# marcusrussi/approximateNN

Hardware: AMD Instinct MI355X
Metric: queries/sec, N=10M d=128 k=10 Q=10k float (query(): hash + candidate gather + L2 + top-k + refine) (higher is better)
Workload: dtype f32; 1 GPU; cfg3: N=10000000 d=128 k=10 tries=10 Q=10000/step float; streams=1, d_short=20, L1=6006, P1=4096, L2=110, P2=64, sum_par_maxes=286

## Files before the change

### approximatenn_amd/_lib.py

```python
import ctypes as C
import os
import subprocess
import threading

CSRC = os.path.join(os.path.dirname(os.path.abspath(__file__)), "csrc")
_libs = {}


class SaveT(C.Structure):
    _fields_ = [("tries", C.c_int), ("n", C.c_size_t), ("k", C.c_size_t),
                ("d_short", C.c_size_t), ("d_long", C.c_size_t),
                ("which_par", C.POINTER(C.POINTER(C.c_size_t))),
                ("par_maxes", C.POINTER(C.c_size_t)), ("graph", C.POINTER(C.c_size_t)),
                ("row_means", C.c_void_p), ("bases", C.c_void_p)]


def build(verbose=False):
    cmd = ["make", "-j4", "-C", CSRC, "all"]
    if not verbose:
        cmd.insert(1, "-s")
    subprocess.check_call(cmd)


def reload_env():
# ... 120 lines not shown
    lib.annhip_stream_open.restype = vp
    lib.annhip_stream_open.argtypes = [vp, sz, C.c_int]
    lib.annhip_stream_submit.restype = C.c_long
    lib.annhip_stream_submit.argtypes = [vp, sz, vp, C.c_int]
    lib.annhip_stream_collect.restype = C.c_int
    lib.annhip_stream_collect.argtypes = [vp, C.c_long, vp, vp]
    lib.annhip_stream_close.argtypes = [vp]
    lib.annhip_key_bytes.restype = sz
    lib.annhip_key_bytes.argtypes = []
    lib.annhip_stream_create_reserving.restype = vp
    lib.annhip_stream_create_reserving.argtypes = [C.c_int]
    lib.annhip_stream_destroy.argtypes = [vp]
    lib.annhip_sh_codes.argtypes = [vp, vp, sz, vp, sz, sz, u32p]
    lib.annhip_sh_stage1.argtypes = [vp, vp, sz, vp, C.c_int, u32p, vp, u32p, u32p]
    lib.annhip_sh_merge_finalize.argtypes = [vp, vp, C.c_int, sz, sz, sz, vp, u32p, u32p, vp]
    lib.annhip_sh_exact1_begin.argtypes = [vp, vp, sz, vp, C.c_int, u32p, u32p, sz, u32p, u32p, vp]
    lib.annhip_sh_exact1_end.argtypes = [vp, vp, sz, sz, sz, sz, u32p, u32p, vp, u32p, vp, u32p, vp]
    lib.annhip_sh_stage2.argtypes = [vp, vp, sz, vp, C.c_int, u32p, vp, u32p]
    lib.annhip_sh_final.argtypes = [vp, vp, C.c_int, sz, sz, sz, u32p, vp, vp, u32p, vp]
    lib.annhip_stage1_rows.argtypes = [vp, sz, vp, C.c_int, u32p, u32p, sz, u32p, vp]
    lib.annhip_stage2_rows_list.argtypes = [vp, sz, vp, C.c_int, u32p, sz, u32p, vp, u32p, vp]
    lib.annhip_exact_select.argtypes = [vp, C.c_int, sz, u32p, vp, u32p, u32p, vp]
    lib.annhip_test_sort_rows.argtypes = [sz, sz, sz, u32p, vp, vp, u32p, u32p, vp, vp, C.c_int]
    lib.annhip_recall_ranks.argtypes = [sz, sz, sz, vp, sz, vp, vp, C.c_int, vp]
    lib.annhip_recall_ranks_host.argtypes = [sz, sz, sz, vp, sz, vp, vp, C.c_int, vp]
    lib.annhip_exact_knn.restype = C.c_int
    lib.annhip_exact_knn.argtypes = [sz, sz, sz, vp, sz, vp, C.c_int, vp, vp]
    lib.annhip_exact_knn_filtered.restype = C.c_int
    lib.annhip_exact_knn_filtered.argtypes = [sz, sz, sz, vp, sz, vp, C.c_int, u32p, vp, vp]
    lib.annhip_exact_knn_tagged.restype = C.c_int
    lib.annhip_exact_knn_tagged.argtypes = [sz, sz, sz, vp, sz, vp, C.c_int, vp, vp, vp, vp, vp, vp]
    lib.annhip_index_exact_query_tagged.restype = C.c_int
    lib.annhip_index_exact_query_tagged.argtypes = [vp, sz, vp, C.c_int, vp, vp, vp, vp]
    lib.annhip_exact_knn_host.restype = C.c_int
    lib.annhip_exact_knn_host.argtypes = [sz, sz, sz, vp, sz, vp, C.c_int, vp, vp]
    lib.annhip_index_exact_query.restype = C.c_int
    lib.annhip_index_exact_query.argtypes = [vp, sz, vp, C.c_int, vp, vp]
    lib.annhip_checksum_dev.restype = C.c_ulonglong
    lib.annhip_checksum_dev.argtypes = [vp, sz, vp]
    lib.annhip_index_checksum.restype = C.c_ulonglong
    lib.annhip_index_checksum.argtypes = [vp]
    lib.annhip_profile.argtypes = [vp, C.c_int]
    lib.annhip_stats.argtypes = [vp, C.POINTER(C.c_double * 8), C.c_int]
    lib.annhip_stage_ms.argtypes = [vp, C.POINTER(C.c_double * 6)]
    lib.annhip_cache_clear.argtypes = []
    lib.annhip_fingerprint_ms.restype = C.c_double
# ... 19 lines not shown
    lib.query_gpu.argtypes = [C.POINTER(SaveT), vp, sz, vp, C.POINTER(vp)]
    lib.precomp_gpu.restype = C.POINTER(sz)
    lib.precomp_gpu.argtypes = [sz, sz, sz, vp, C.c_int, sz, sz, sz, sz, C.POINTER(SaveT), C.POINTER(vp)]
    _libs[prec] = lib
    return lib


EXPORTED = ["gpu_init", "gpu_cleanup", "register_cleanup", "query_gpu", "precomp_gpu", "annhip_precision", "annhip_layout_code",
            "annhip_index_create", "annhip_index_destroy", "annhip_index_info", "annhip_index_set_stream", "annhip_index_set_gather_pieces", "annhip_index_set_gather_slots", "annhip_index_set_fixed",
            "annhip_index_set_rows", "annhip_index_rows", "annhip_index_set_prune", "annhip_index_prune",
            "annhip_index_set_probe", "annhip_index_probe", "annhip_probe_bits",
            "annhip_index_set_filter", "annhip_index_filter_count", "annhip_filter_pack", "annhip_exact_knn_filtered",
            "annhip_index_set_tags", "annhip_index_has_tags", "annhip_query_tagged", "annhip_exact_knn_tagged",
            "annhip_index_exact_query_tagged",
            "annhip_query_k", "annhip_index_max_query_k", "annhip_index_exact_query_k",
            "annhip_query_radius", "annhip_index_exact_query_radius", "annhip_radius_trim",
            "annhip_rerank", "annhip_index_rerank",
            "annhip_index_append", "annhip_index_reserve_tail", "annhip_index_tail", "annhip_index_copy_rows", "annhip_index_drop_tail",
            "annhip_index_hash_tail", "annhip_index_tail_hashed",
            "annhip_index_fixed", "annhip_index_copy_words",
            "annhip_index_export", "annhip_index_reshard", "annhip_save_write", "annhip_save_read", "annhip_precomp_index", "annhip_precomp_begin", "annhip_precomp_info", "annhip_precomp_init_merged", "annhip_precomp_hash",
            "annhip_precomp_try", "annhip_precomp_merge", "annhip_precomp_graph", "annhip_precomp_finish", "annhip_query", "annhip_workspace_create", "annhip_workspace_destroy", "annhip_query_on", "annhip_query_slice", "annhip_stream_open", "annhip_stream_submit", "annhip_stream_collect", "annhip_stream_close",
            "annhip_key_bytes", "annhip_stream_create_reserving", "annhip_stream_destroy", "annhip_sh_codes", "annhip_sh_stage1", "annhip_sh_merge_finalize", "annhip_sh_exact1_begin", "annhip_sh_exact1_end", "annhip_sh_stage2",
            "annhip_sh_final", "annhip_stage1_rows", "annhip_stage2_rows_list", "annhip_exact_select", "annhip_test_sort_rows",
            "annhip_recall_ranks", "annhip_recall_ranks_host", "annhip_exact_knn", "annhip_exact_knn_host", "annhip_index_exact_query", "annhip_checksum_dev", "annhip_index_checksum", "annhip_profile", "annhip_stats", "annhip_stage_ms",
            "annhip_cache_clear", "annhip_fingerprint_ms", "annhip_cache_drop", "annhip_cache_size", "annhip_reload_env",
            "annhip_synth_randnorm", "annhip_synth_reset", "annhip_host_profile", "annhip_host_stats",
            "annhip_host_shards", "annhip_host_stats_shard", "annhip_set_devices"]
DISPATCH_EXPORTED = ["precomp", "query", "free_save"]


_libc = C.CDLL("libc.so.6")
_libc.initstate.restype = C.c_void_p
_libc.initstate.argtypes = [C.c_uint, C.c_void_p, C.c_size_t]
_libc.setstate.restype = C.c_void_p
_libc.setstate.argtypes = [C.c_void_p]
_RAND_WORDS = (1, 8, 16, 32, 64)
_restored = []


_park_lock = threading.Lock()
_park_depth = 0
_park_old = None


class park_random:

# ... 33 lines not shown
```

### approximatenn_amd/csrc/ann_host.hip

```cpp
#include <hip/hip_fp16.h>
#include <hip/hip_runtime.h>
#include <math.h>
#include <stdio.h>
#include <stdlib.h>
#include <string.h>
#include <time.h>

#include <algorithm>
#include <limits>
#include <mutex>
#include <vector>

#include "../../include/algg.h"
#include "../../include/ann_hip.h"
#include "../../include/gpu_comp.h"
#include "ann_hostpool.h"
#include "ann_precomp_kernels.h"
#include "ann_query_kernels.h"
#include "ann_probe_kernels.h"
#include "ann_recall_kernels.h"
#include "ann_exact_kernels.h"
#include "ann_filter_kernels.h"
#include "ann_tag_kernels.h"
#include "ann_kq_kernels.h"
// ... 978 lines not shown
      if constexpr (D <= 0) {
        allow_lds(codes_kernel<D>, smem);
        hipLaunchKernelGGL(codes_kernel<D>, dim3(grid), dim3(64 * wpb), smem, s, P, (int)Q, y, codes, zero_me);
      }
    });
  }
  HIPCHECK(hipGetLastError());
}

static int stage1_waves(u32 P1, double own_frac) {
  int w = (int)(P1 / ANN_S1_CHUNK);
  if (w < 1) w = 1;
  if (w > 4) w = 4;
  if (own_frac <= 0.5) w = 1;
  if (env().s1_waves) w = env().s1_waves;
  return w;
}
static int stage1_cap(int W, int K1) {
  int cap = 256;
  if (cap < W * K1) cap = W * K1;
  if (cap < K1 + 128) cap = K1 + 128;
  return (cap + 63) & ~63;
}
static size_t stage1_lds_bytes(const QParams &P, int W, int K1, int cap, u32 tail_len = 0) {
  size_t b = sizeof(Key) * (size_t)W * cap + 2 * sizeof(Key) * (size_t)W * K1 + sizeof(TryInfo) * (size_t)P.T +
             sizeof(u32 *) * (size_t)W * ANN_WAVE + sizeof(u32) * (size_t)W * ANN_S1_CHUNK +
             sizeof(u32) * (size_t)W * ANN_WAVE + sizeof(u32) * (size_t)P.T + sizeof(int) * (size_t)W + sizeof(u32) * 4 +
             3 * sizeof(u32) * (size_t)tail_len;
  b = (b + 15) & ~(size_t)15;
  b += sizeof(FT) * (size_t)tail_len;
  b = (b + 15) & ~(size_t)15;
  if (d_needs_lds_row(P.d)) b += sizeof(FT) * (size_t)P.d * (1 + W);
  return b;
}

__global__ void zero_u32_kernel(u32 *p) { *p = 0; }

__global__ void sum_u32_kernel(size_t count, const u32 *__restrict__ v, unsigned long long *out) {
  unsigned long long acc = 0;
  for (size_t e = (size_t)blockIdx.x * blockDim.x + threadIdx.x; e < count; e += (size_t)gridDim.x * blockDim.x)
    acc += v[e];
#pragma unroll
  for (int s = 32; s >= 1; s >>= 1) acc += __shfl_xor(acc, s);
  if (lane_id() == 0) atomicAdd(out, acc);
}

static EventPair s1_prof_begin(annhip_index *ix, hipStream_t s) {
  EventPair ev;
// ... 2 lines not shown
    HIPCHECK(hipEventCreate(&ev.b));
  } else {
    ev = ix->ev_free.back();
    ix->ev_free.pop_back();
  }
  HIPCHECK(hipEventRecord(ev.a, s));
  return ev;
}
static void s1_prof_end(annhip_index *ix, EventPair ev, size_t Q, const u32 *nvo, hipStream_t s) {
  HIPCHECK(hipEventRecord(ev.b, s));
  ix->ev_used.push_back(ev);
  if (ix->profile == 1) sum_u32_kernel<<<grid_for(Q, 256, 64), 256, 0, s>>>(Q, nvo, ix->d_rows);
}

static void launch_stage1(annhip_index *ix, const QParams &P, size_t Q, const FT *y, int alias,
                          const u32 *codes, FT *cand_d, u32 *cand_i, u32 *nvt, u32 *nvo, hipStream_t s,
                          const std::vector<TryInfo> &h_tries, int use_seg, FusedTail F = FusedTail{0, 0, NULL, NULL, NULL, NULL, NULL, NULL, NULL},
                          Key *cand_key = NULL, int pieces = 1, int slots = 0, size_t qstride = 0, int keys = 0,
                          bool bracket = true) {
  const int kq = (int)(qstride ? qstride : Q);
  if (!Q) return;
  if (keys && F.enabled) die("launch_stage1: a preselection has no fused tail");
  const int K1 = keys ? keys : P.k + 1, W = stage1_waves(P.P1, (double)(P.hi - P.lo) / (double)P.n), cap = stage1_cap(W, K1);
  const size_t smem = stage1_lds_bytes(P, W, K1, cap, F.enabled == 1 ? F.len2 : 0);
  u32 runs_used = 0;
  for (int t = 0; t < P.T; t++)
    for (int yy = 0; yy <= P.ds; yy++)
      if (h_tries[t].off + (u32)yy * h_tries[t].pm < P.P1) runs_used++;
  unsigned max_grid = 0xFFFFFFFFu;
  if (slots > 0) max_grid = std::max(1u, (unsigned)device_cus() * 4u * (unsigned)slots / (unsigned)W);
  EventPair ev;
  const bool prof = ix && ix->profile && bracket;
  if (prof) ev = s1_prof_begin(ix, s);
  const size_t np = (size_t)std::max(1, std::min(pieces, 64)), per = (Q + np - 1) / np;
  with_value(QueryLayouts{}, layout_code(P.d), [&](auto dd) {
    with_rows(P, [&](auto rt) {
      auto launch = [&](auto sg, auto fu) {
        constexpr int D = decltype(dd)::value, SG = decltype(sg)::value;
        constexpr bool FU = decltype(fu)::value;
        using RT = typename decltype(rt)::type;
        allow_lds(stage1_select_kernel<D, SG, FU, RT>, smem);
        for (size_t a = 0; a < Q; a += per) {
          QParams Pp = P;
          Pp.q0 = (u32)a, Pp.qn = (u32)std::min(per, Q - a);
          hipLaunchKernelGGL((stage1_select_kernel<D, SG, FU, RT>), dim3(std::min<unsigned>(Pp.qn, max_grid)), dim3(64 * W), smem,
                             s, Pp, kq, y, alias, codes, K1, cap, runs_used, cand_d, cand_i, nvt, nvo, F, cand_key);
        }
      };
      if (use_seg == 2) launch(Int<2>{}, std::false_type{});
      else if (use_seg && F.enabled == 1) launch(Int<1>{}, std::true_type{});
      else if (use_seg) launch(Int<1>{}, std::false_type{});
      else if (F.enabled == 1) launch(Int<0>{}, std::true_type{});
      else launch(Int<0>{}, std::false_type{});
    });
  });
  HIPCHECK(hipGetLastError());
  if (prof) s1_prof_end(ix, ev, Q, nvo, s);
  if (ix) ix->s1_launches += 1;
}

#ifdef USE_FLOAT
static void launch_prune_rescore(annhip_index *ix, const QParams &P, size_t Q, const FT *y, int kp, const FT *pre_d,
                                 const u32 *pre_i, const u32 *nvt, u32 *nvo, u32 *top_i, FT *top_d, u32 *fl, u32 *d_fcount,
                                 hipStream_t s) {
  if (!Q) return;
  if (kp < P.k + 1 || kp > ANN_PRUNE_KMAX || P.k + 1 > 32) die("launch_prune_rescore: preselection size out of range");
  PruneArgs A = {};
  A.points = P.points, A.y = y, A.pre_d = pre_d, A.pre_i = pre_i, A.nv_tot = nvt, A.nv_own = nvo;
  A.top_id = top_i, A.top_dist = top_d, A.flist = fl, A.fcount = d_fcount;
  A.exact_total = ix->d_rows + 2, A.uncertified = ix->d_rows + 4;
// ... 1018 lines not shown
                          NULL, ids_dev, reinterpret_cast<FT *>(dist_dev), ix->profile == 1 ? ix->d_rows + 8 : NULL, ix->stream);
}

extern "C" void annhip_exact_select(annhip_index *ix, int stage, size_t nq, uint32_t *ids_dev, ftype *dist_dev,
                                    const uint32_t *qidx_dev, uint32_t *out_id_dev, ftype *out_dist_dev) {
  const u32 L = stage == 1 ? ix->L1 : ix->L2, len = stage == 1 ? ix->Lc1 : ix->Lc2;
  launch_exact_select(L, len, len, (int)ix->k, nq, ids_dev, reinterpret_cast<FT *>(dist_dev), qidx_dev, 0,
                      out_id_dev, reinterpret_cast<FT *>(out_dist_dev), (int)ix->k, 0, ix->stream, NULL, NULL, 1024, 0,
                      TieArgs{NULL, NULL, (int)ix->k + 1, ix->d_rows + 3, 1});
}

extern "C" void annhip_test_sort_rows(size_t L, size_t k, size_t nq, uint32_t *ids_dev, ftype *dist_dev,
                                      const ftype *cand_d_dev, const uint32_t *cand_i_dev, uint32_t *out_id_dev,
                                      ftype *out_dist_dev, unsigned long long *resolved_dev, int derive) {
  gpu_init();
  const u32 len = (u32)ann_need_len(L, k);
  launch_exact_select((u32)L, len, len, (int)k, nq, ids_dev, reinterpret_cast<FT *>(dist_dev), NULL, 0, out_id_dev,
                      reinterpret_cast<FT *>(out_dist_dev), (int)k, 0, NULL, NULL, NULL, 1024, 0,
                      TieArgs{reinterpret_cast<const FT *>(cand_d_dev), cand_i_dev, (int)k + 1, resolved_dev,
                              cand_d_dev ? 0 : derive});
  HIPCHECK(hipStreamSynchronize(NULL));
}

extern "C" void *annhip_stream_create_reserving(int reserve) {
  gpu_init();
  int dev = 0;
  hipDeviceProp_t prop;
  if (hipGetDevice(&dev) != hipSuccess || hipGetDeviceProperties(&prop, dev) != hipSuccess) return NULL;
  const int ncu = prop.multiProcessorCount;
  if (reserve < 0 || reserve >= ncu) return NULL;
  std::vector<uint32_t> mask((ncu + 31) / 32, 0u);
  for (int cu = 0; cu < ncu - reserve; cu++) mask[cu / 32] |= 1u << (cu % 32);
  hipStream_t st = NULL;
  if (hipExtStreamCreateWithCUMask(&st, (uint32_t)mask.size(), mask.data()) != hipSuccess) {
    (void)hipGetLastError();
    return NULL;
  }
  return st;
}
extern "C" void annhip_stream_destroy(void *hip_stream) {
  if (hip_stream) (void)hipStreamDestroy((hipStream_t)hip_stream);
}

extern "C" size_t annhip_key_bytes(void) { return sizeof(Key); }

extern "C" void annhip_sh_codes(annhip_index *ix, void *hip_stream, size_t Q, const ftype *y_dev, size_t q_lo, size_t q_hi,
// ... 1574 lines not shown
```

### approximatenn_amd/csrc/ann_query_kernels.h

```cpp
#pragma once
#include <type_traits>

#include "ann_device.h"
#include "ann_tie.h"

#ifndef ANN_ROWS_INFLIGHT
#define ANN_ROWS_INFLIGHT 1
#endif

struct TryInfo {
  const u32 *tab;
  const uint2 *seg;
  const uint4 *segx;
  u32 pm;
  u32 off;
  u32 end;
  u32 magic;
};

struct QParams {
  const FT *points;
  const TryInfo *tries;
  const u32 *graph;
  const FT *means;
  const FT *bases;
  u32 n, lo, hi;
  int d, k, T, ds;
  u32 L1, P1, Lc1, L2, Lc2;
  u32 q0, qn;
  u32 fixed;
  const RN *points_h = nullptr;
};

#define ANN_S1_CHUNK 1024
#ifndef ANN_S1_PREFETCH
#define ANN_S1_PREFETCH 3
#endif
#ifndef ANN_S1_PREFETCH_OC
#define ANN_S1_PREFETCH_OC 2
#endif

template <bool NT>
__device__ __forceinline__ VT load_row_chunk(const VT *p) {
  if constexpr (NT) {
    typedef FT native_vec __attribute__((ext_vector_type(ANN_VEC)));
    native_vec v = __builtin_nontemporal_load(reinterpret_cast<const native_vec *>(p));
    return __builtin_bit_cast(VT, v);
  } else {
    return *p;
  }
}

template <typename RT>
__device__ __forceinline__ const RT *q_rows(const QParams &P) {
  if constexpr (std::is_same<RT, FT>::value) return P.points;
  else return P.points_h;
}
template <typename RT, bool NT>
__device__ __forceinline__ typename RowRaw<RT>::T load_row_raw(const RT *row, int ci) {
// ... 231 lines not shown
  w[0] = zs | (co << 8) | (ca << 16);
  const u32 *row = tab + b * pm + zs;
#pragma unroll
  for (int j = 0; j < ANN_SEGX_INLINE; j++) w[1 + j] = (u32)j < co ? row[j] : ANN_ID_NONE;
  segx[2 * b] = make_uint4(w[0], w[1], w[2], w[3]);
  segx[2 * b + 1] = make_uint4(w[4], w[5], w[6], w[7]);
}

struct SelState {
  Key *kbuf, *kout;
  int kcnt, K1, cap;
  Key tau;
};

__device__ __forceinline__ void sel_shrink(SelState &S) {
  wave_lds_sync();
  const int m = wave_select_smallest(S.kbuf, S.kcnt, S.K1, S.kout);
  for (int i = lane_id(); i < m; i += ANN_WAVE) S.kbuf[i] = S.kout[i];
  if (m == S.K1) S.tau = S.kout[S.K1 - 1];
  S.kcnt = m;
  wave_lds_sync();
}

struct FoldPlan {
  int L, sL;
  int h[5], odd[5], sprev[5];
  __device__ __forceinline__ explicit FoldPlan(int d) {
    int s = d;
    L = 0;
    while (L < 5 && s > 16) {
      sprev[L] = s, h[L] = s >> 1, odd[L] = s & 1;
      s >>= 1;
      L++;
    }
    sL = s;
    if (sL > 64) L = 0;
  }
};

template <int LV, typename RT>
__device__ __forceinline__ void gather_fold(const QParams &P, const FoldPlan &fp, const u32 *list, int cnt, int alias, u32 x,
                                            const FT *yrow, SelState &S) {
  const RT *rows = q_rows<RT>(P);
  constexpr int NL = 1 << LV;
  const int lane = lane_id(), d = P.d, sL = fp.sL, rpw = ANN_WAVE / sL;
  const int g = lane / sL, z = lane - g * sL;
// ... 68 lines not shown
#pragma unroll
    for (int l = 0; l < LV; l++)
#pragma unroll
      for (int i = 0; i < NL; i += 2 << l) e[i] = e[i] + (e[i + (1 << l)] + (i == 0 ? gx[l] : zero));
    FT v = e[0];
    for (int s = sL; s >> 1; s >>= 1) {
      const int h = s >> 1;
      const FT o = __shfl(v, lane + h);
      FT gg = zero;
      if (s & 1) gg = __shfl(v, lane - z + s - 1);
      if (z < h) v = v + (o + (z == 0 ? gg : zero));
    }
    const Key key = key_make(v, id);
    const bool pass = act && z == 0 && key_less(key, S.tau);
    const u64 mm = __ballot(pass);
    if (mm) {
      if (pass) S.kbuf[S.kcnt + mask_rank(mm)] = key;
      S.kcnt += __popcll(mm);
      if (S.kcnt + rpw > S.cap) sel_shrink(S);
    }
  }
}

template <int D, typename RT = FT>
__device__ __forceinline__ void gather_select(const QParams &P, const u32 *list, int cnt, int alias, u32 x,
                                              const VT (&a)[RowChunks<D>::C],
                                              const FT *yq, FT *scratch, SelState &S, const FT *yrow = NULL) {
  const int lane = lane_id();
  const RT *rows = q_rows<RT>(P);
  typedef typename RowRaw<RT>::T RR;
  if constexpr (D > 0) {
    typedef RowLay<D> L;
    constexpr int PF = ANN_S1_PREFETCH;
    const int p = lane % L::LPR, g = lane / L::LPR;
    RR buf[PF][L::C];
    u32 idb[PF];
#pragma unroll
    for (int s = 0; s < PF; s++) {
      const int first = s * L::RPW;
      idb[s] = 0;
      if (first < cnt) {
        idb[s] = list[first + g < cnt ? first + g : first];
        const RT *rp = rows + (size_t)(idb[s] - P.lo) * D;
#pragma unroll
        for (int c = 0; c < L::C; c++) buf[s][c] = load_row_raw<RT, true>(rp, p + c * L::LPR);
      }
    }
    for (int base = 0; base < cnt; base += PF * L::RPW) {
#pragma unroll
      for (int s = 0; s < PF; s++) {
        const int cur = base + s * L::RPW;
        if (cur < cnt) {
          const u32 id = idb[s];
          const bool act = cur + g < cnt && !(alias && id == x);
          const FT dist = row_reduce<D, ROW_SQDIFF>(a, buf[s]);
          const int nb = cur + PF * L::RPW;
          if (nb < cnt) {
            idb[s] = list[nb + g < cnt ? nb + g : nb];
            const RT *rp = rows + (size_t)(idb[s] - P.lo) * D;
#pragma unroll
            for (int c = 0; c < L::C; c++) buf[s][c] = load_row_raw<RT, true>(rp, p + c * L::LPR);
          }
          const Key key = key_make(dist, id);
          const bool pass = act && p == 0 && key_less(key, S.tau);
          const u64 mm = __ballot(pass);
          if (mm) {
            if (pass) S.kbuf[S.kcnt + mask_rank(mm)] = key;
            S.kcnt += __popcll(mm);
            if (S.kcnt + L::RPW > S.cap) sel_shrink(S);
          }
        }
      }
    }
  } else if constexpr (OcCode<D>::FOLD > 0) {
    const FoldPlan fp(P.d);
    gather_fold<OcCode<D>::FOLD, RT>(P, fp, list, cnt, alias, x, yrow, S);
  } else if constexpr (D < 0 && !OcCode<D>::GEN) {
    constexpr int C = OcCode<D>::C, OC = OcCode<D>::OC;
    constexpr int PF = ANN_S1_PREFETCH_OC;
    const OcLanes<D> ol(P.d, lane);
    const int oc = ol.oc, rpw = ol.rpw, g = ol.g, p = ol.p;
    RR buf[PF][C];
    u32 idb[PF];
#pragma unroll
    for (int s = 0; s < PF; s++) {
      const int first = s * rpw;
      idb[s] = 0;
      if (first < cnt) {
        idb[s] = list[(ol.valid && first + g < cnt) ? first + g : first];
        const RT *rp = rows + (size_t)(idb[s] - P.lo) * P.d;
#pragma unroll
        for (int c = 0; c < C; c++) buf[s][c] = oc_load_chunk<D, OcCode<D>::NT_ROWS>(rp, p + c * oc, P.d);
      }
    }
    for (int base = 0; base < cnt; base += PF * rpw) {
#pragma unroll
      for (int s = 0; s < PF; s++) {
        const int cur = base + s * rpw;
        if (cur < cnt) {
          const u32 id = idb[s];
          const bool act = ol.valid && cur + g < cnt && !(alias && id == x);
          const FT dist = row_reduce_oc<C, ROW_SQDIFF, OC>(a, buf[s], oc, p, oc_tree_len<D>(P.d));
          const int nb = cur + PF * rpw;
          if (nb < cnt) {
            idb[s] = list[(ol.valid && nb + g < cnt) ? nb + g : nb];
            const RT *rp = rows + (size_t)(idb[s] - P.lo) * P.d;
#pragma unroll
            for (int c = 0; c < C; c++) buf[s][c] = oc_load_chunk<D, OcCode<D>::NT_ROWS>(rp, p + c * oc, P.d);
          }
          const Key key = key_make(dist, id);
          const bool pass = act && p == 0 && key_less(key, S.tau);
          const u64 mm = __ballot(pass);
          if (mm) {
            if (pass) S.kbuf[S.kcnt + mask_rank(mm)] = key;
            S.kcnt += __popcll(mm);
            if (S.kcnt + rpw > S.cap) sel_shrink(S);
          }
        }
      }
    }
  } else {
    for (int r = 0; r < cnt; r++) {
      const u32 id = list[r];
      if (alias && id == x) continue;
      const FT dist = row_reduce_generic<ROW_SQDIFF>(P.d, yq, rows + (size_t)(id - P.lo) * P.d, scratch);
      const Key key = key_make(dist, id);
      if (key_less(key, S.tau)) {
        if (lane == 0) S.kbuf[S.kcnt] = key;
        S.kcnt++;
        if (S.kcnt + 1 > S.cap) sel_shrink(S);
      }
    }
  }
  wave_lds_sync();
}

template <int D, typename IdOut, typename RT = FT>
__device__ __forceinline__ u32 stage2_in_workgroup(const QParams &P, u32 x, int alias, const VT (&a)[RowChunks<D>::C],
                                                   const FT *yq, FT *scratch, const Key *top, int k, u32 len2,
                                                   u32 *t_ids, u32 *t_slot, u32 *t_gid, FT *t_dist, u32 *cnt2p,
// ... 246 lines not shown
        if (exact_total) atomicAdd(exact_total, 1ull);
      }
    } else {
      for (int t = lane; t < k; t += ANN_WAVE) {
        out_ids[(size_t)x * k + t] = t < m ? (IdOut)key_id(S.kout[t]) : (IdOut)P.n;
        out_dist[(size_t)x * k + t] = t < m ? key_dist(S.kout[t]) : ft_inf();
      }
    }
    if (rows_done && lane == 0) atomicAdd(&rows_done[(x & 63u) * 8u], (unsigned long long)cnts[1]);
  }
}

struct FusedTail {
  int enabled;
  u32 len2;
  size_t *out_ids;
  FT *out_dist;
  u32 *flist, *fcount;
  unsigned long long *exact_total;
  u32 *top_id;
  FT *top_dist;
};

template <int D, int SEG, bool FUSED, typename RT>
__global__ __launch_bounds__(256) void stage1_select_kernel(QParams P, int Q, const FT *__restrict__ y,
                                                            int alias, const u32 *__restrict__ codes,
                                                            int K1, int cap, u32 runs_used,
                                                            FT *__restrict__ cand_dist,
                                                            u32 *__restrict__ cand_id,
                                                            u32 *__restrict__ nv_tot,
                                                            u32 *__restrict__ nv_own, FusedTail F,
                                                            Key *__restrict__ cand_key) {
  extern __shared__ __attribute__((aligned(16))) unsigned char smem[];
  const int lane = lane_id(), w = threadIdx.x >> 6, W = blockDim.x >> 6;
  unsigned char *sp = smem;
  Key *kbuf_all = reinterpret_cast<Key *>(sp);           sp += sizeof(Key) * (size_t)W * cap;
  Key *kout_all = reinterpret_cast<Key *>(sp);           sp += sizeof(Key) * (size_t)W * K1;
  Key *mbuf = reinterpret_cast<Key *>(sp);               sp += sizeof(Key) * (size_t)W * K1;
  TryInfo *tries = reinterpret_cast<TryInfo *>(sp);      sp += sizeof(TryInfo) * (size_t)P.T;
  const u32 **rptr_all = reinterpret_cast<const u32 **>(sp);  sp += sizeof(u32 *) * (size_t)W * ANN_WAVE;
  u32 *list_all = reinterpret_cast<u32 *>(sp);           sp += sizeof(u32) * (size_t)W * ANN_S1_CHUNK;
  u32 *pref_all = reinterpret_cast<u32 *>(sp);           sp += sizeof(u32) * (size_t)W * ANN_WAVE;
  u32 *qcode = reinterpret_cast<u32 *>(sp);              sp += sizeof(u32) * (size_t)P.T;
  int *mcnt = reinterpret_cast<int *>(sp);               sp += sizeof(int) * (size_t)W;
  u32 *cnts = reinterpret_cast<u32 *>(sp);               sp += sizeof(u32) * 4;
  const size_t tl = FUSED ? F.len2 : 0;
  u32 *t_ids = reinterpret_cast<u32 *>(sp);              sp += sizeof(u32) * tl;
  u32 *t_slot = reinterpret_cast<u32 *>(sp);             sp += sizeof(u32) * tl;
  u32 *t_gid = reinterpret_cast<u32 *>(sp);              sp += sizeof(u32) * tl;
  sp = smem + (((sp - smem) + 15) & ~(size_t)15);
  FT *t_dist = reinterpret_cast<FT *>(sp);               sp += sizeof(FT) * tl;
  sp = smem + (((sp - smem) + 15) & ~(size_t)15);
  FT *yq = reinterpret_cast<FT *>(sp);
  u32 *list = list_all + (size_t)w * ANN_S1_CHUNK;
  u32 *pref = pref_all + (size_t)w * ANN_WAVE;
  const u32 **rptr = rptr_all + (size_t)w * ANN_WAVE;

  for (u32 xi = blockIdx.x; xi < P.qn; xi += gridDim.x) {
  const u32 x = xi + P.q0;
  if (xi != blockIdx.x) __syncthreads();
  for (int i = threadIdx.x; i < P.T; i += blockDim.x) {
    tries[i] = P.tries[i];
    qcode[i] = P.fixed ? codes[(size_t)x * P.T + i] : codes[(size_t)i * Q + x];
  }
  if (threadIdx.x < 4) cnts[threadIdx.x] = 0;
  if constexpr (D == 0 || OcCode<D>::GEN)
    for (int z = threadIdx.x; z < P.d; z += blockDim.x) yq[z] = y[(size_t)x * P.d + z];
  __syncthreads();

  SelState S;
  S.kbuf = kbuf_all + (size_t)w * cap, S.kout = kout_all + (size_t)w * K1;
  S.kcnt = 0, S.K1 = K1, S.cap = cap, S.tau = key_max();
  FT *scratch = yq + (size_t)(1 + w) * P.d;
  u32 vtot = 0, vown = 0;

  VT a[RowChunks<D>::C];
  if constexpr (D > 0) {
    typedef RowLay<D> L;
    const VT *yp = reinterpret_cast<const VT *>(y + (size_t)x * D) + (lane % L::LPR);
#pragma unroll
    for (int c = 0; c < L::C; c++) a[c] = yp[c * L::LPR];
  } else if constexpr (D < 0 && !OcCode<D>::GEN) {
    const OcLanes<D> ol(P.d, lane);
#pragma unroll
    for (int c = 0; c < OcCode<D>::C; c++) a[c] = oc_load_chunk<D, false>(y + (size_t)x * P.d, ol.p + c * ol.oc, P.d);
  }

  int cnt = 0;
  if constexpr (SEG == 2) {
    const u32 ds1 = (u32)P.ds + 1u;
    const u32 per = (runs_used + W - 1) / W;
    const u32 r0 = min(runs_used, (u32)w * per), r1 = min(runs_used, r0 + per);
    for (u32 rb = r0; rb < r1; rb += ANN_WAVE) {
      const u32 r = rb + lane;
      u32 c = 0, va = 0;
// ... 101 lines not shown
    for (u32 base = s0; base < s1; base += ANN_WAVE) {
      const u32 j = base + lane;
      u32 id = ANN_ID_NONE;
      if (j < s1) id = slot_id(tries, qcode, j, ti);
      const bool ok = id < P.n && !(alias && id == x);
      const bool own = ok && id >= P.lo && id < P.hi;
      vtot += __popcll(__ballot(ok));
      const u64 mm = __ballot(own);
      if (own) list[cnt + mask_rank(mm)] = id;
      cnt += __popcll(mm);
      if (cnt + ANN_WAVE > ANN_S1_CHUNK) {
        wave_lds_sync();
        vown += cnt;
        gather_select<D, RT>(P, list, cnt, alias, x, a, yq, scratch, S, y + (size_t)x * P.d);
        cnt = 0;
      }
    }
  }
  wave_lds_sync();
  vown += cnt;
  gather_select<D, RT>(P, list, cnt, alias, x, a, yq, scratch, S, y + (size_t)x * P.d);

  {
    const int m = wave_select_smallest(S.kbuf, S.kcnt, K1, S.kout);
    for (int i = lane; i < m; i += ANN_WAVE) mbuf[(size_t)w * K1 + i] = S.kout[i];
    if (lane == 0) {
      mcnt[w] = m;
      atomicAdd(&cnts[0], vtot);
      atomicAdd(&cnts[1], vown);
    }
  }
  __syncthreads();
  if (w == 0) {
    int total = 0;
    for (int ww = 0; ww < W; ww++) {
      const int m = mcnt[ww];
      for (int i = lane; i < m; i += ANN_WAVE) S.kbuf[total + i] = mbuf[(size_t)ww * K1 + i];
      total += m;
    }
    wave_lds_sync();
    const int m = wave_select_smallest(S.kbuf, total, K1, S.kout);
    if constexpr (!FUSED) {
      if (cand_key) {
        for (int i = lane; i < K1; i += ANN_WAVE) cand_key[(size_t)x * K1 + i] = i < m ? S.kout[i] : key_make(ft_inf(), ANN_ID_NONE);
      } else {
        for (int i = lane; i < K1; i += ANN_WAVE) {
          cand_dist[(size_t)x * K1 + i] = i < m ? key_dist(S.kout[i]) : ft_inf();
          cand_id[(size_t)x * K1 + i] = i < m ? key_id(S.kout[i]) : ANN_ID_NONE;
        }
      }
      if (lane == 0) {
        nv_tot[x] = cnts[0];
        nv_own[x] = cnts[1];
      }
      if (F.enabled == 2) {
        const int k = K1 - 1;
        bool bad = m < k;
        for (int t = lane; t + 1 < m; t += ANN_WAVE)
          if (ft_bits(key_dist(S.kout[t])) == ft_bits(key_dist(S.kout[t + 1]))) bad = true;
        if (m >= k && !(key_dist(S.kout[k - 1]) < ft_inf())) bad = true;
        if (P.L1 > P.P1 && cnts[0] >= P.P1) bad = true;
        if (__ballot(bad) != 0) {
          if (lane == 0) {
            F.flist[atomicAdd(F.fcount, 1u)] = x;
            if (F.exact_total) atomicAdd(F.exact_total, 1ull);
          }
        } else {
          for (int t = lane; t < k; t += ANN_WAVE) {
            F.top_id[(size_t)x * k + t] = key_id(S.kout[t]);
            F.top_dist[(size_t)x * k + t] = key_dist(S.kout[t]);
          }
        }
      }
    } else {
      const int k = K1 - 1;
      bool bad = m < k;
      for (int t = lane; t + 1 < m; t += ANN_WAVE)
        if (ft_bits(key_dist(S.kout[t])) == ft_bits(key_dist(S.kout[t + 1]))) bad = true;
      if (m >= k && !(key_dist(S.kout[k - 1]) < ft_inf())) bad = true;
      if (P.L1 > P.P1 && cnts[0] >= P.P1) bad = true;
      const bool reject = __ballot(bad) != 0;
      if (reject && cand_dist)
        for (int i = lane; i < K1; i += ANN_WAVE) {
          cand_dist[(size_t)x * K1 + i] = i < m ? key_dist(S.kout[i]) : ft_inf();
          cand_id[(size_t)x * K1 + i] = i < m ? key_id(S.kout[i]) : ANN_ID_NONE;
        }
      if (lane == 0) {
        cnts[3] = reject ? 1u : 0u;
        if (reject) {
          F.flist[atomicAdd(F.fcount, 1u)] = x;
          atomicAdd(F.exact_total, 1ull);
        }
      }
    }
  }
  if constexpr (FUSED) {
  __syncthreads();
  if (cnts[3]) {
    if (threadIdx.x == 0) nv_own[x] = cnts[1];
    continue;
  }
  {
    const u32 cnt2 = stage2_in_workgroup<D, size_t, RT>(P, x, alias, a, yq, scratch, kout_all ,
                                                    K1 - 1, F.len2, t_ids, t_slot, t_gid, t_dist, &cnts[2], F.out_ids, F.out_dist);
    if (threadIdx.x == 0) nv_own[x] = cnts[1] + cnt2;
  }
  }
  }
}

#ifndef ANN_BK_TILE_CHUNKS
#define ANN_BK_TILE_CHUNKS 1024
#endif
#ifndef ANN_BK_MEMBERS
#define ANN_BK_MEMBERS 1
#endif
#ifndef ANN_BK_WAVES
#define ANN_BK_WAVES 4
#endif
#ifndef ANN_BK_WAVES_HI
#define ANN_BK_WAVES_HI 8
#endif
#define ANN_BK_MAX_RUNS 64
template <int D, bool HI>
__global__ __launch_bounds__(64 * (HI ? ANN_BK_WAVES_HI : ANN_BK_WAVES)) void stage1_bucket_kernel(QParams P, int K1, u32 list_cap, u32 mgroup,
                                                            FT *__restrict__ cand_dist, u32 *__restrict__ cand_id,
                                                            u32 *__restrict__ nv_tot, u32 *__restrict__ nv_own,
                                                            u32 brem, u32 bmod) {
  typedef RowLay<D> L;
  extern __shared__ __attribute__((aligned(16))) unsigned char smem[];
// ... 577 lines not shown
```

### include/ann_hip.h

```cpp
#ifndef APPROXNN_HIP_ANN_HIP_H
#define APPROXNN_HIP_ANN_HIP_H
#include <stddef.h>
#include <stdint.h>
#include "ann.h"
#ifdef __cplusplus
extern "C" {
#endif

typedef struct annhip_index annhip_index;

const char *annhip_precision(void);
int annhip_layout_code(size_t d);

annhip_index *annhip_index_create(const save_t *save, const ftype *points, int points_on_device,
                                  size_t row_lo, size_t row_hi);
void annhip_index_destroy(annhip_index *ix);
void annhip_index_info(const annhip_index *ix, size_t out[12]);
void annhip_index_set_stream(annhip_index *ix, void *hip_stream);
void annhip_index_set_gather_pieces(annhip_index *ix, int pieces);
void annhip_index_set_gather_slots(annhip_index *ix, int waves_per_simd);
void annhip_index_set_fixed(annhip_index *ix, int fixed);
enum { ANNHIP_PROBE_ALL = -1 };
int annhip_index_set_probe(annhip_index *ix, int pair_bits);
int annhip_index_probe(const annhip_index *ix);
// ... 91 lines not shown
                            uint32_t *flist_dev, uint32_t *rows_id_dev, ftype *rows_dist_dev);
void annhip_sh_exact1_end(annhip_index *ix, void *hip_stream, size_t ycnt, size_t q_lo, size_t qs, size_t fcap,
                          const uint32_t *flist_dev, uint32_t *rows_id_dev, ftype *rows_dist_dev,
                          uint32_t *top_id_all_dev, ftype *top_dist_all_dev, uint32_t *top_id_dev,
                          ftype *top_dist_dev);
void annhip_sh_stage2(annhip_index *ix, void *hip_stream, size_t ycnt, const ftype *y_dev, int alias,
                      const uint32_t *top_id_all_dev, ftype *dist_out_dev, uint32_t *flagged_dev);
void annhip_sh_final(annhip_index *ix, void *hip_stream, int ndev, size_t ycnt, size_t q_lo, size_t qs,
                     const uint32_t *top_id_dev, const ftype *top_dist_dev, const ftype *dist_in_dev,
                     uint32_t *out_id_dev, ftype *out_dist_dev);
void annhip_stage1_rows(annhip_index *ix, size_t ycnt, const ftype *y_dev, int alias,
                        const uint32_t *codes_dev, const uint32_t *qidx_dev, size_t nq,
                        uint32_t *ids_dev, ftype *dist_dev);
void annhip_stage2_rows_list(annhip_index *ix, size_t ycnt, const ftype *y_dev, int alias, const uint32_t *qidx_dev,
                             size_t nq, const uint32_t *top_id_dev, const ftype *top_dist_dev, uint32_t *ids_dev,
                             ftype *dist_dev);
void annhip_exact_select(annhip_index *ix, int stage, size_t nq, uint32_t *ids_dev, ftype *dist_dev,
                         const uint32_t *qidx_dev, uint32_t *out_id_dev, ftype *out_dist_dev);

void annhip_test_sort_rows(size_t L, size_t k, size_t nq, uint32_t *ids_dev, ftype *dist_dev, const ftype *cand_d_dev,
                           const uint32_t *cand_i_dev, uint32_t *out_id_dev, ftype *out_dist_dev,
                           unsigned long long *resolved_dev, int derive);

unsigned long long annhip_checksum_dev(const void *dev_ptr, size_t nbytes, void *hip_stream);
unsigned long long annhip_index_checksum(annhip_index *ix);

void annhip_recall_ranks(size_t n, size_t d, size_t k, const ftype *points_dev, size_t ycnt, const ftype *y_dev,
                         const size_t *guess_dev, int self, unsigned long long *ranks_dev);
void annhip_recall_ranks_host(size_t n, size_t d, size_t k, const ftype *points, size_t ycnt, const ftype *y,
                              const size_t *guess, int self, unsigned long long *ranks_host);

int annhip_exact_knn(size_t n, size_t d, size_t k, const ftype *points_dev, size_t ycnt, const ftype *y_dev,
                     int self, size_t *ids_dev, ftype *dists_dev);
int annhip_exact_knn_filtered(size_t n, size_t d, size_t k, const ftype *points_dev, size_t ycnt, const ftype *y_dev,
                              int self, const uint32_t *bits_dev, size_t *ids_dev, ftype *dists_dev);
int annhip_exact_knn_tagged(size_t n, size_t d, size_t k, const ftype *points_dev, size_t ycnt, const ftype *y_dev,
                            int self, const uint32_t *tags_dev, const uint32_t *bits_dev ,
                            const uint32_t *qmask_dev, const uint32_t *qvalue_dev, size_t *ids_dev, ftype *dists_dev);
int annhip_exact_knn_host(size_t n, size_t d, size_t k, const ftype *points, size_t ycnt, const ftype *y,
                          int self, size_t *ids, ftype *dists);
int annhip_index_exact_query(annhip_index *ix, size_t ycnt, const ftype *y_dev, int alias,
                             size_t *ids_dev, ftype *dists_dev);
int annhip_index_exact_query_tagged(annhip_index *ix, size_t ycnt, const ftype *y_dev, int alias,
                                    const uint32_t *qmask_dev, const uint32_t *qvalue_dev, size_t *ids_dev,
                                    ftype *dists_dev);
int annhip_index_exact_query_k(annhip_index *ix, size_t ycnt, const ftype *y_dev, int alias, size_t kq,
// ... 32 lines not shown
```

Baseline: 11.55 million queries/s.

## Keep stage-1 top-k selection in wave registers instead of LDS buffers

Stage-1 candidate selection now keeps a running top-K1 inside wave registers (one or two keys per lane with a threshold) for layouts and K1 up to twice the wave width, instead of appending passing keys to a per-wave LDS buffer and periodically shrinking it. The LDS reservation shrinks because the per-wave candidate buffers go away, which may raise occupancy. The cross-wave merge re-offers other waves' results into wave 0's register state. A test entry point and kernel are added to check register selection against the LDS path. Each offer now pays a register top-k insertion cost instead of an LDS append.

```diff
diff --git a/approximatenn_amd/_lib.py b/approximatenn_amd/_lib.py
--- a/approximatenn_amd/_lib.py
+++ b/approximatenn_amd/_lib.py
@@ -166,6 +166,8 @@
     lib.annhip_stage2_rows_list.argtypes = [vp, sz, vp, C.c_int, u32p, sz, u32p, vp, u32p, vp]
     lib.annhip_exact_select.argtypes = [vp, C.c_int, sz, u32p, vp, u32p, u32p, vp]
     lib.annhip_test_sort_rows.argtypes = [sz, sz, sz, u32p, vp, vp, u32p, u32p, vp, vp, C.c_int]
+    lib.annhip_test_select.restype = C.c_int
+    lib.annhip_test_select.argtypes = [sz, u32p, vp, u32p, sz, C.c_int, C.c_int, vp, u32p]
     lib.annhip_recall_ranks.argtypes = [sz, sz, sz, vp, sz, vp, vp, C.c_int, vp]
     lib.annhip_recall_ranks_host.argtypes = [sz, sz, sz, vp, sz, vp, vp, C.c_int, vp]
     lib.annhip_exact_knn.restype = C.c_int
@@ -231,7 +233,7 @@
             "annhip_index_export", "annhip_index_reshard", "annhip_save_write", "annhip_save_read", "annhip_precomp_index", "annhip_precomp_begin", "annhip_precomp_info", "annhip_precomp_init_merged", "annhip_precomp_hash",
             "annhip_precomp_try", "annhip_precomp_merge", "annhip_precomp_graph", "annhip_precomp_finish", "annhip_query", "annhip_workspace_create", "annhip_workspace_destroy", "annhip_query_on", "annhip_query_slice", "annhip_stream_open", "annhip_stream_submit", "annhip_stream_collect", "annhip_stream_close",
             "annhip_key_bytes", "annhip_stream_create_reserving", "annhip_stream_destroy", "annhip_sh_codes", "annhip_sh_stage1", "annhip_sh_merge_finalize", "annhip_sh_exact1_begin", "annhip_sh_exact1_end", "annhip_sh_stage2",
-            "annhip_sh_final", "annhip_stage1_rows", "annhip_stage2_rows_list", "annhip_exact_select", "annhip_test_sort_rows",
+            "annhip_sh_final", "annhip_stage1_rows", "annhip_stage2_rows_list", "annhip_exact_select", "annhip_test_sort_rows", "annhip_test_select",
             "annhip_recall_ranks", "annhip_recall_ranks_host", "annhip_exact_knn", "annhip_exact_knn_host", "annhip_index_exact_query", "annhip_checksum_dev", "annhip_index_checksum", "annhip_profile", "annhip_stats", "annhip_stage_ms",
             "annhip_cache_clear", "annhip_fingerprint_ms", "annhip_cache_drop", "annhip_cache_size", "annhip_reload_env",
             "annhip_synth_randnorm", "annhip_synth_reset", "annhip_host_profile", "annhip_host_stats",
diff --git a/approximatenn_amd/csrc/ann_host.hip b/approximatenn_amd/csrc/ann_host.hip
--- a/approximatenn_amd/csrc/ann_host.hip
+++ b/approximatenn_amd/csrc/ann_host.hip
@@ -1024,8 +1024,9 @@
   if (cap < K1 + 128) cap = K1 + 128;
   return (cap + 63) & ~63;
 }
-static size_t stage1_lds_bytes(const QParams &P, int W, int K1, int cap, u32 tail_len = 0) {
-  size_t b = sizeof(Key) * (size_t)W * cap + 2 * sizeof(Key) * (size_t)W * K1 + sizeof(TryInfo) * (size_t)P.T +
+static size_t stage1_lds_bytes(const QParams &P, int W, int K1, int cap, u32 tail_len = 0, bool regs = false) {
+  size_t b = sizeof(Key) * (regs ? 0 : (size_t)W * cap) + sizeof(Key) * (size_t)(regs ? 1 : W) * K1 +
+             sizeof(Key) * (size_t)W * K1 + sizeof(TryInfo) * (size_t)P.T +
              sizeof(u32 *) * (size_t)W * ANN_WAVE + sizeof(u32) * (size_t)W * ANN_S1_CHUNK +
              sizeof(u32) * (size_t)W * ANN_WAVE + sizeof(u32) * (size_t)P.T + sizeof(int) * (size_t)W + sizeof(u32) * 4 +
              3 * sizeof(u32) * (size_t)tail_len;
@@ -1074,7 +1075,8 @@
   if (!Q) return;
   if (keys && F.enabled) die("launch_stage1: a preselection has no fused tail");
   const int K1 = keys ? keys : P.k + 1, W = stage1_waves(P.P1, (double)(P.hi - P.lo) / (double)P.n), cap = stage1_cap(W, K1);
-  const size_t smem = stage1_lds_bytes(P, W, K1, cap, F.enabled == 1 ? F.len2 : 0);
+  const bool regs = K1 <= ANN_SEL_REGS_KMAX && sel_regs_code(layout_code(P.d));
+  const size_t smem = stage1_lds_bytes(P, W, K1, cap, F.enabled == 1 ? F.len2 : 0, regs);
   u32 runs_used = 0;
   for (int t = 0; t < P.T; t++)
     for (int yy = 0; yy <= P.ds; yy++)
@@ -1087,17 +1089,25 @@
   const size_t np = (size_t)std::max(1, std::min(pieces, 64)), per = (Q + np - 1) / np;
   with_value(QueryLayouts{}, layout_code(P.d), [&](auto dd) {
     with_rows(P, [&](auto rt) {
-      auto launch = [&](auto sg, auto fu) {
+      auto launch_sel = [&](auto sg, auto fu, auto rg) {
         constexpr int D = decltype(dd)::value, SG = decltype(sg)::value;
-        constexpr bool FU = decltype(fu)::value;
+        constexpr bool FU = decltype(fu)::value, RG = decltype(rg)::value;
         using RT = typename decltype(rt)::type;
-        allow_lds(stage1_select_kernel<D, SG, FU, RT>, smem);
+        allow_lds(stage1_select_kernel<D, SG, FU, RT, RG>, smem);
         for (size_t a = 0; a < Q; a += per) {
           QParams Pp = P;
           Pp.q0 = (u32)a, Pp.qn = (u32)std::min(per, Q - a);
-          hipLaunchKernelGGL((stage1_select_kernel<D, SG, FU, RT>), dim3(std::min<unsigned>(Pp.qn, max_grid)), dim3(64 * W), smem,
+          hipLaunchKernelGGL((stage1_select_kernel<D, SG, FU, RT, RG>), dim3(std::min<unsigned>(Pp.qn, max_grid)), dim3(64 * W), smem,
                              s, Pp, kq, y, alias, codes, K1, cap, runs_used, cand_d, cand_i, nvt, nvo, F, cand_key);
         }
+      };
+      auto launch = [&](auto sg, auto fu) {
+        if constexpr (sel_regs_layout<decltype(dd)::value>()) {
+          if (regs) return launch_sel(sg, fu, std::true_type{});
+        } else if (regs) {
+          die("launch_stage1: register selection chosen for a layout without one");
+        }
+        launch_sel(sg, fu, std::false_type{});
       };
       if (use_seg == 2) launch(Int<2>{}, std::false_type{});
       else if (use_seg && F.enabled == 1) launch(Int<1>{}, std::true_type{});
@@ -2162,6 +2172,27 @@
   HIPCHECK(hipStreamSynchronize(NULL));
 }
 
+extern "C" int annhip_test_select(size_t ns, const uint32_t *off_dev, const ftype *dist_dev, const uint32_t *id_dev, size_t K1,
+                                  int W, int lds, ftype *out_dist_dev, uint32_t *out_id_dev) {
+  gpu_init();
+  if (K1 < 1 || K1 > 256 || W < 1 || W > 4 || (!lds && K1 > ANN_SEL_REGS_KMAX)) return -1;
+  if (!ns) return 0;
+  const int cap = stage1_cap(W, (int)K1);
+  const size_t smem = sizeof(Key) * (lds ? (size_t)W * cap : 0) + sizeof(Key) * (size_t)(lds ? W : 1) * K1 +
+                      sizeof(Key) * (size_t)W * K1 + sizeof(int) * (size_t)W;
+  auto launch = [&](auto rg) {
+    constexpr bool RG = decltype(rg)::value;
+    allow_lds(test_select_kernel<RG>, smem);
+    hipLaunchKernelGGL(test_select_kernel<RG>, dim3((unsigned)ns), dim3(64 * W), smem, NULL, off_dev,
+                       reinterpret_cast<const FT *>(dist_dev), id_dev, (int)K1, cap, reinterpret_cast<FT *>(out_dist_dev), out_id_dev);
+  };
+  if (lds) launch(std::false_type{});
+  else launch(std::true_type{});
+  HIPCHECK(hipGetLastError());
+  HIPCHECK(hipStreamSynchronize(NULL));
+  return 0;
+}
+
 extern "C" void *annhip_stream_create_reserving(int reserve) {
   gpu_init();
   int dev = 0;
diff --git a/approximatenn_amd/csrc/ann_query_kernels.h b/approximatenn_amd/csrc/ann_query_kernels.h
--- a/approximatenn_amd/csrc/ann_query_kernels.h
+++ b/approximatenn_amd/csrc/ann_query_kernels.h
@@ -35,6 +35,9 @@
 #define ANN_S1_CHUNK 1024
 #ifndef ANN_S1_PREFETCH
 #define ANN_S1_PREFETCH 3
+#endif
+#ifndef ANN_S1_PREFETCH_NARROW
+#define ANN_S1_PREFETCH_NARROW 3
 #endif
 #ifndef ANN_S1_PREFETCH_OC
 #define ANN_S1_PREFETCH_OC 2
@@ -312,6 +315,96 @@
   wave_lds_sync();
 }
 
+struct SelRegs {
+  Key lo, hi;
+  int K1;
+  Key tau;
+};
+constexpr bool sel_regs_code(int code) {
+  return code > 0 || (code < 0 && code != ANN_D_FOLD2 && code != ANN_D_FOLD3 && code != ANN_D_FOLD4 && code != ANN_D_FOLD4G &&
+                      code != ANN_D_FOLD5G);
+}
+template <int D>
+constexpr bool sel_regs_layout() {
+  static_assert(sel_regs_code(D) == (D > 0 || (D < 0 && !OcCode<D>::GEN && OcCode<D>::FOLD == 0)), "the two forms of the rule differ");
+  return sel_regs_code(D);
+}
+#define ANN_SEL_REGS_KMAX (2 * ANN_WAVE)
+template <bool REGS>
+struct SelOf {
+  typedef SelState T;
+};
+template <>
+struct SelOf<true> {
+  typedef SelRegs T;
+};
+
+__device__ __forceinline__ void sel_offer(SelState &S, Key key, bool pass, int rpw) {
+  const u64 mm = __ballot(pass);
+  if (mm) {
+    if (pass) S.kbuf[S.kcnt + mask_rank(mm)] = key;
+    S.kcnt += __popcll(mm);
+    if (S.kcnt + rpw > S.cap) sel_shrink(S);
+  }
+}
+__device__ __forceinline__ void sel_offer(SelRegs &S, Key key, bool pass, int) {
+  const u64 mm = __ballot(pass);
+  if (mm) {
+    if (S.K1 <= ANN_WAVE) wave_topk_offer(S.lo, S.tau, key, mm, S.K1);
+    else wave_topk_offer2(S.lo, S.hi, S.tau, key, mm, S.K1);
+  }
+}
+
+__device__ __forceinline__ void sel_init(SelState &S, Key *kbuf, Key *kout, int K1, int cap) {
+  S.kbuf = kbuf, S.kout = kout;
+  S.kcnt = 0, S.K1 = K1, S.cap = cap, S.tau = key_max();
+}
+__device__ __forceinline__ void sel_init(SelRegs &S, Key *, Key *, int K1, int) {
+  S.lo = S.hi = S.tau = key_max();
+  S.K1 = K1;
+}
+
+__device__ __forceinline__ int sel_wave_result(SelState &S, Key *out) {
+  const int m = wave_select_smallest(S.kbuf, S.kcnt, S.K1, S.kout);
+  for (int i = lane_id(); i < m; i += ANN_WAVE) out[i] = S.kout[i];
+  return m;
+}
+__device__ __forceinline__ int sel_wave_result(SelRegs &S, Key *out) {
+  int m = __popcll(__ballot(!key_eq(S.lo, key_max())));
+  if (S.K1 > ANN_WAVE) m += __popcll(__ballot(!key_eq(S.hi, key_max())));
+  m = min(m, S.K1);
+  const int lane = lane_id();
+  if (lane < m) out[lane] = S.lo;
+  if (ANN_WAVE + lane < m) out[ANN_WAVE + lane] = S.hi;
+  return m;
+}
+
+__device__ __forceinline__ int sel_merge(SelState &S, const Key *mbuf, const int *mcnt, int W, Key *kout) {
+  const int lane = lane_id();
+  int total = 0;
+  for (int ww = 0; ww < W; ww++) {
+    const int m = mcnt[ww];
+    for (int i = lane; i < m; i += ANN_WAVE) S.kbuf[total + i] = mbuf[(size_t)ww * S.K1 + i];
+    total += m;
+  }
+  wave_lds_sync();
+  return wave_select_smallest(S.kbuf, total, S.K1, kout);
+}
+__device__ __forceinline__ int sel_merge(SelRegs &S, const Key *mbuf, const int *mcnt, int W, Key *kout) {
+  const int lane = lane_id();
+  for (int ww = 1; ww < W; ww++) {
+    const int mw = mcnt[ww];
+    for (int base = 0; base < mw; base += ANN_WAVE) {
+      const bool in = base + lane < mw;
+      const Key key = in ? mbuf[(size_t)ww * S.K1 + base + lane] : key_max();
+      sel_offer(S, key, in && key_less(key, S.tau), 0);
+    }
+  }
+  const int m = sel_wave_result(S, kout);
+  wave_lds_sync();
+  return m;
+}
+
 struct FoldPlan {
   int L, sL;
   int h[5], odd[5], sprev[5];
@@ -426,16 +519,16 @@
   }
 }
 
-template <int D, typename RT = FT>
+template <int D, typename RT = FT, typename ST = SelState>
 __device__ __forceinline__ void gather_select(const QParams &P, const u32 *list, int cnt, int alias, u32 x,
                                               const VT (&a)[RowChunks<D>::C],
-                                              const FT *yq, FT *scratch, SelState &S, const FT *yrow = NULL) {
+                                              const FT *yq, FT *scratch, ST &S, const FT *yrow = NULL) {
   const int lane = lane_id();
   const RT *rows = q_rows<RT>(P);
   typedef typename RowRaw<RT>::T RR;
   if constexpr (D > 0) {
     typedef RowLay<D> L;
-    constexpr int PF = ANN_S1_PREFETCH;
+    constexpr int PF = std::is_same<RT, FT>::value ? ANN_S1_PREFETCH : ANN_S1_PREFETCH_NARROW;
     const int p = lane % L::LPR, g = lane / L::LPR;
     RR buf[PF][L::C];
     u32 idb[PF];
@@ -467,12 +560,7 @@
           }
           const Key key = key_make(dist, id);
           const bool pass = act && p == 0 && key_less(key, S.tau);
-          const u64 mm = __ballot(pass);
-          if (mm) {
-            if (pass) S.kbuf[S.kcnt + mask_rank(mm)] = key;
-            S.kcnt += __popcll(mm);
-            if (S.kcnt + L::RPW > S.cap) sel_shrink(S);
-          }
+          sel_offer(S, key, pass, L::RPW);
         }
       }
     }
@@ -514,12 +602,7 @@
           }
           const Key key = key_make(dist, id);
           const bool pass = act && p == 0 && key_less(key, S.tau);
-          const u64 mm = __ballot(pass);
-          if (mm) {
-            if (pass) S.kbuf[S.kcnt + mask_rank(mm)] = key;
-            S.kcnt += __popcll(mm);
-            if (S.kcnt + rpw > S.cap) sel_shrink(S);
-          }
+          sel_offer(S, key, pass, rpw);
         }
       }
     }
@@ -812,7 +895,7 @@
   FT *top_dist;
 };
 
-template <int D, int SEG, bool FUSED, typename RT>
+template <int D, int SEG, bool FUSED, typename RT, bool REGS>
 __global__ __launch_bounds__(256) void stage1_select_kernel(QParams P, int Q, const FT *__restrict__ y,
                                                             int alias, const u32 *__restrict__ codes,
                                                             int K1, int cap, u32 runs_used,
@@ -824,8 +907,8 @@
   extern __shared__ __attribute__((aligned(16))) unsigned char smem[];
   const int lane = lane_id(), w = threadIdx.x >> 6, W = blockDim.x >> 6;
   unsigned char *sp = smem;
-  Key *kbuf_all = reinterpret_cast<Key *>(sp);           sp += sizeof(Key) * (size_t)W * cap;
-  Key *kout_all = reinterpret_cast<Key *>(sp);           sp += sizeof(Key) * (size_t)W * K1;
+  Key *kbuf_all = reinterpret_cast<Key *>(sp);           sp += sizeof(Key) * (REGS ? 0 : (size_t)W * cap);
+  Key *kout_all = reinterpret_cast<Key *>(sp);           sp += sizeof(Key) * (size_t)(REGS ? 1 : W) * K1;
   Key *mbuf = reinterpret_cast<Key *>(sp);               sp += sizeof(Key) * (size_t)W * K1;
   TryInfo *tries = reinterpret_cast<TryInfo *>(sp);      sp += sizeof(TryInfo) * (size_t)P.T;
   const u32 **rptr_all = reinterpret_cast<const u32 **>(sp);  sp += sizeof(u32 *) * (size_t)W * ANN_WAVE;
@@ -858,9 +941,10 @@
     for (int z = threadIdx.x; z < P.d; z += blockDim.x) yq[z] = y[(size_t)x * P.d + z];
   __syncthreads();
 
-  SelState S;
-  S.kbuf = kbuf_all + (size_t)w * cap, S.kout = kout_all + (size_t)w * K1;
-  S.kcnt = 0, S.K1 = K1, S.cap = cap, S.tau = key_max();
+  static_assert(!REGS || sel_regs_layout<D>(), "this layout's gather has no register selection");
+  typename SelOf<REGS>::T S;
+  Key *const kout = kout_all + (REGS ? 0 : (size_t)w * K1);
+  sel_init(S, kbuf_all + (REGS ? 0 : (size_t)w * cap), kout, K1, cap);
   FT *scratch = yq + (size_t)(1 + w) * P.d;
   u32 vtot = 0, vown = 0;
 
@@ -1008,8 +1092,7 @@
   gather_select<D, RT>(P, list, cnt, alias, x, a, yq, scratch, S, y + (size_t)x * P.d);
 
   {
-    const int m = wave_select_smallest(S.kbuf, S.kcnt, K1, S.kout);
-    for (int i = lane; i < m; i += ANN_WAVE) mbuf[(size_t)w * K1 + i] = S.kout[i];
+    const int m = sel_wave_result(S, mbuf + (size_t)w * K1);
     if (lane == 0) {
       mcnt[w] = m;
       atomicAdd(&cnts[0], vtot);
@@ -1018,21 +1101,14 @@
   }
   __syncthreads();
   if (w == 0) {
-    int total = 0;
-    for (int ww = 0; ww < W; ww++) {
-      const int m = mcnt[ww];
-      for (int i = lane; i < m; i += ANN_WAVE) S.kbuf[total + i] = mbuf[(size_t)ww * K1 + i];
-      total += m;
-    }
-    wave_lds_sync();
-    const int m = wave_select_smallest(S.kbuf, total, K1, S.kout);
+    const int m = sel_merge(S, mbuf, mcnt, W, kout);
     if constexpr (!FUSED) {
       if (cand_key) {
-        for (int i = lane; i < K1; i += ANN_WAVE) cand_key[(size_t)x * K1 + i] = i < m ? S.kout[i] : key_make(ft_inf(), ANN_ID_NONE);
+        for (int i = lane; i < K1; i += ANN_WAVE) cand_key[(size_t)x * K1 + i] = i < m ? kout[i] : key_make(ft_inf(), ANN_ID_NONE);
       } else {
         for (int i = lane; i < K1; i += ANN_WAVE) {
-          cand_dist[(size_t)x * K1 + i] = i < m ? key_dist(S.kout[i]) : ft_inf();
-          cand_id[(size_t)x * K1 + i] = i < m ? key_id(S.kout[i]) : ANN_ID_NONE;
+          cand_dist[(size_t)x * K1 + i] = i < m ? key_dist(kout[i]) : ft_inf();
+          cand_id[(size_t)x * K1 + i] = i < m ? key_id(kout[i]) : ANN_ID_NONE;
         }
       }
       if (lane == 0) {
@@ -1043,8 +1119,8 @@
         const int k = K1 - 1;
         bool bad = m < k;
         for (int t = lane; t + 1 < m; t += ANN_WAVE)
-          if (ft_bits(key_dist(S.kout[t])) == ft_bits(key_dist(S.kout[t + 1]))) bad = true;
-        if (m >= k && !(key_dist(S.kout[k - 1]) < ft_inf())) bad = true;
+          if (ft_bits(key_dist(kout[t])) == ft_bits(key_dist(kout[t + 1]))) bad = true;
+        if (m >= k && !(key_dist(kout[k - 1]) < ft_inf())) bad = true;
         if (P.L1 > P.P1 && cnts[0] >= P.P1) bad = true;
         if (__ballot(bad) != 0) {
           if (lane == 0) {
@@ -1053,8 +1129,8 @@
           }
         } else {
           for (int t = lane; t < k; t += ANN_WAVE) {
-            F.top_id[(size_t)x * k + t] = key_id(S.kout[t]);
-            F.top_dist[(size_t)x * k + t] = key_dist(S.kout[t]);
+            F.top_id[(size_t)x * k + t] = key_id(kout[t]);
+            F.top_dist[(size_t)x * k + t] = key_dist(kout[t]);
           }
         }
       }
@@ -1062,14 +1138,14 @@
       const int k = K1 - 1;
       bool bad = m < k;
       for (int t = lane; t + 1 < m; t += ANN_WAVE)
-        if (ft_bits(key_dist(S.kout[t])) == ft_bits(key_dist(S.kout[t + 1]))) bad = true;
-      if (m >= k && !(key_dist(S.kout[k - 1]) < ft_inf())) bad = true;
+        if (ft_bits(key_dist(kout[t])) == ft_bits(key_dist(kout[t + 1]))) bad = true;
+      if (m >= k && !(key_dist(kout[k - 1]) < ft_inf())) bad = true;
       if (P.L1 > P.P1 && cnts[0] >= P.P1) bad = true;
       const bool reject = __ballot(bad) != 0;
       if (reject && cand_dist)
         for (int i = lane; i < K1; i += ANN_WAVE) {
-          cand_dist[(size_t)x * K1 + i] = i < m ? key_dist(S.kout[i]) : ft_inf();
-          cand_id[(size_t)x * K1 + i] = i < m ? key_id(S.kout[i]) : ANN_ID_NONE;
+          cand_dist[(size_t)x * K1 + i] = i < m ? key_dist(kout[i]) : ft_inf();
+          cand_id[(size_t)x * K1 + i] = i < m ? key_id(kout[i]) : ANN_ID_NONE;
         }
       if (lane == 0) {
         cnts[3] = reject ? 1u : 0u;
@@ -1092,6 +1168,40 @@
     if (threadIdx.x == 0) nv_own[x] = cnts[1] + cnt2;
   }
   }
+  }
+}
+
+template <bool REGS>
+__global__ __launch_bounds__(256) void test_select_kernel(const u32 *__restrict__ off, const FT *__restrict__ dist,
+                                                          const u32 *__restrict__ id, int K1, int cap,
+                                                          FT *__restrict__ out_dist, u32 *__restrict__ out_id) {
+  extern __shared__ __attribute__((aligned(16))) unsigned char smem[];
+  const int lane = lane_id(), w = threadIdx.x >> 6, W = blockDim.x >> 6;
+  unsigned char *sp = smem;
+  Key *kbuf_all = reinterpret_cast<Key *>(sp);  sp += sizeof(Key) * (REGS ? 0 : (size_t)W * cap);
+  Key *kout_all = reinterpret_cast<Key *>(sp);  sp += sizeof(Key) * (size_t)(REGS ? 1 : W) * K1;
+  Key *mbuf = reinterpret_cast<Key *>(sp);      sp += sizeof(Key) * (size_t)W * K1;
+  int *mcnt = reinterpret_cast<int *>(sp);
+  typename SelOf<REGS>::T S;
+  Key *const kout = kout_all + (REGS ? 0 : (size_t)w * K1);
+  sel_init(S, kbuf_all + (REGS ? 0 : (size_t)w * cap), kout, K1, cap);
+  const u32 b = blockIdx.x, s0 = off[b], s1 = off[b + 1];
+  for (u32 base = s0 + (u32)w * ANN_WAVE; base < s1; base += (u32)W * ANN_WAVE) {
+    const u32 i = base + lane;
+    const bool in = i < s1;
+    const Key key = in ? key_make(dist[i], id[i]) : key_max();
+    sel_offer(S, key, in && key_less(key, S.tau), ANN_WAVE);
+  }
+  wave_lds_sync();
+  const int mw = sel_wave_result(S, mbuf + (size_t)w * K1);
+  if (lane == 0) mcnt[w] = mw;
+  __syncthreads();
+  if (w == 0) {
+    const int m = sel_merge(S, mbuf, mcnt, W, kout);
+    for (int i = lane; i < K1; i += ANN_WAVE) {
+      out_dist[(size_t)b * K1 + i] = i < m ? key_dist(kout[i]) : ft_inf();
+      out_id[(size_t)b * K1 + i] = i < m ? key_id(kout[i]) : ANN_ID_NONE;
+    }
   }
 }
 
diff --git a/include/ann_hip.h b/include/ann_hip.h
--- a/include/ann_hip.h
+++ b/include/ann_hip.h
@@ -137,6 +137,9 @@
                            const uint32_t *cand_i_dev, uint32_t *out_id_dev, ftype *out_dist_dev,
                            unsigned long long *resolved_dev, int derive);
 
+int annhip_test_select(size_t ns, const uint32_t *off_dev, const ftype *dist_dev, const uint32_t *id_dev, size_t K1, int W,
+                       int lds, ftype *out_dist_dev, uint32_t *out_id_dev);
+
 unsigned long long annhip_checksum_dev(const void *dev_ptr, size_t nbytes, void *hip_stream);
 unsigned long long annhip_index_checksum(annhip_index *ix);
 
```

New measurement: 12.43 million queries/s (median of 6 runs). 7.6% higher.
